# vadimkantorov/convasr

Hardware: AMD Instinct MI355X
Metric: audio-seconds/sec/node (fwd+bwd+CTC) at bs64x15s (higher is better)
Workload: dtype bf16

## Files before the change

### convasr_amd/csrc/conv1x1.hip

```cpp
#include "conv_v2_common.h"

#define C11_THREADS 256
#define C11_BM 128
#define C11_STAGE (2 * C11_BM * ROW_BYTES)

struct C11Args {
	const void* x; const void* w; void* y; const float* bias; double* stats;
	int Cin, Cout, CoutPad;
	int64_t M;
	int accumulate;
};

template <typename I, int NS> __device__ __forceinline__ void conv1x1_tile(const C11Args& p, const int mtile, const int ntile, char* const smem) {
	constexpr int MI = 4, NB = 4;
	const int tid = threadIdx.x, lane = tid & 63;
	const int wave = __builtin_amdgcn_readfirstlane(tid >> 6);
	const int r16 = lane & 15, kb = lane >> 4, wm = wave >> 1, wn = wave & 1;

	const int m0 = mtile * C11_BM, co0 = ntile * BN;
	const int64_t M = p.M;

	const int row_bytes = p.Cin * 2;
	const v4i32 xsrc = make_srd(p.x, (unsigned)(M * row_bytes));
	const v4i32 wsrc = make_srd(p.w, (unsigned)(p.CoutPad * row_bytes));
	const unsigned lds_base = (unsigned)(size_t)(__attribute__((address_space(3))) char*)smem;
	const int n_cib = p.Cin >> 6;

	const int plane = v2s_src_offset(lane, row_bytes);
	auto issue = [&](int cib, int stage) {
		const unsigned dst = lds_base + stage * C11_STAGE;
		const int xbase = m0 * row_bytes + cib * 128, wbase = co0 * row_bytes + cib * 128;
#pragma unroll
		for (int j = 0; j < 4; ++j) {
			const int u = wave + 4 * j;
			dma16(xsrc, __builtin_amdgcn_readfirstlane(dst + u * 1024), xbase + u * 8 * row_bytes + plane);
			dma16(wsrc, __builtin_amdgcn_readfirstlane(dst + C11_BM * ROW_BYTES + u * 1024), wbase + u * 8 * row_bytes + plane);
		}
	};

	f32x4 acc[MI][NB];
#pragma unroll
	for (int i = 0; i < MI; ++i)
#pragma unroll
		for (int j = 0; j < NB; ++j) acc[i][j] = f32x4{0.f, 0.f, 0.f, 0.f};

	typedef unsigned u32x4 __attribute__((ext_vector_type(4)));
	typedef const __attribute__((address_space(3))) u32x4* lds_u4;
	const int kb4 = kb << 4;
	auto lane_off = [&](int row) { return (unsigned)((row << 7) + (kb4 ^ ((row << 4) & 0x60))); };
	const unsigned xa0 = lds_base + lane_off(wm * 64 + r16), wa0 = lds_base + C11_BM * ROW_BYTES + lane_off(wn * 64 + r16);

	if (NS == 2) {
		issue(0, 0);
		asm volatile("s_waitcnt vmcnt(0)" ::: "memory");
	}
	for (int cib = 0; cib < n_cib; ++cib) {
		if (NS == 1) {
			if (cib) __builtin_amdgcn_s_barrier();
			issue(cib, 0);
			asm volatile("s_waitcnt vmcnt(0)" ::: "memory");
		}
		__builtin_amdgcn_s_barrier();
		if (NS == 2 && cib + 1 < n_cib) issue(cib + 1, (cib + 1) & 1);
		const unsigned so = NS == 2 ? (cib & 1) * C11_STAGE : 0u;
#pragma unroll
		for (int ks = 0; ks < 2; ++ks) {
			u32x4 a[MI], b[NB];
			const unsigned xa = (xa0 + so) ^ (ks << 6), wa = (wa0 + so) ^ (ks << 6);
#pragma unroll
			for (int i = 0; i < MI; ++i) { a[i] = *(lds_u4)(size_t)(xa + i * 2048); b[i] = *(lds_u4)(size_t)(wa + i * 2048); }
#pragma unroll
			for (int i = 0; i < MI; ++i)
#pragma unroll
				for (int j = 0; j < NB; ++j) acc[i][j] = Mma16<I>::run(a[i], b[j], acc[i][j]);
		}
		if (NS == 2) asm volatile("s_waitcnt vmcnt(0)" ::: "memory");
	}
	__syncthreads();

	constexpr int OPITCH = BN * 2 + 16;
	char* const otile = smem;
	float* const red = reinterpret_cast<float*>(smem + C11_BM * OPITCH);
	const bool full = m0 + C11_BM <= M;
#pragma unroll
	for (int ni = 0; ni < NB; ++ni) {
		const int col = wn * 64 + ni * 16 + r16, co = co0 + col;
		const float bias = (p.bias && co < p.Cout) ? p.bias[co] : 0.f;
		float s1 = 0.f, s2 = 0.f;
#pragma unroll
		for (int mi = 0; mi < MI; ++mi) {
#pragma unroll
			for (int g = 0; g < 4; ++g) {
				const int row = wm * 64 + mi * 16 + kb * 4 + g;
				const float val = acc[mi][ni][g] + bias;
				if (p.stats && (full || m0 + row < M)) { s1 += val; s2 += val * val; }
				Elem<I>::store(reinterpret_cast<I*>(otile + row * OPITCH) + col, val);
			}
		}
		if (p.stats) {
			s1 += __shfl_xor(s1, 16, 64); s2 += __shfl_xor(s2, 16, 64);
			s1 += __shfl_xor(s1, 32, 64); s2 += __shfl_xor(s2, 32, 64);
			if (kb == 0) { red[(0 * 2 + wm) * BN + col] = s1; red[(1 * 2 + wm) * BN + col] = s2; }
		}
	}
	__syncthreads();
	if (p.stats && tid < BN && co0 + tid < p.Cout) {
		double* const prow = p.stats + (int64_t)mtile * 2 * p.Cout;
		prow[co0 + tid] = (double)red[(0 * 2 + 0) * BN + tid] + (double)red[(0 * 2 + 1) * BN + tid];
		prow[p.Cout + co0 + tid] = (double)red[(1 * 2 + 0) * BN + tid] + (double)red[(1 * 2 + 1) * BN + tid];
	}
	I* const yb = reinterpret_cast<I*>(p.y);
	constexpr int OCH = BN / 8;
#pragma unroll
	for (int it = 0; it < C11_BM * OCH / C11_THREADS; ++it) {
		const int e = tid + it * C11_THREADS, row = e / OCH, ch = e % OCH;
		const int64_t m = (int64_t)m0 + row;
		if (m < M) {
			uint4 val = *reinterpret_cast<const uint4*>(otile + row * OPITCH + ch * 16);
			uint4* const dst = reinterpret_cast<uint4*>(yb + m * p.Cout + co0 + ch * 8);
			if (p.accumulate) {
				float a[8], o[8];
				unpack16<I>(val, a);
				unpack16<I>(*dst, o);
				val = make_uint4(pack16<I>(a[0] + o[0], a[1] + o[1]), pack16<I>(a[2] + o[2], a[3] + o[3]), pack16<I>(a[4] + o[4], a[5] + o[5]), pack16<I>(a[6] + o[6], a[7] + o[7]));
			}
			*dst = val;
		}
	}
}

template <typename I, int NS> __global__ __launch_bounds__(C11_THREADS, NS == 1 ? 4 : 2) void conv1x1_kernel(ConvParams p) {
	extern __shared__ __attribute__((aligned(16))) char smem[];
	const int v = xcd_remap(blockIdx.x, p.total_tiles);
	C11Args a;
	a.x = p.x; a.w = p.w; a.y = p.y; a.bias = p.bias; a.stats = p.stats; a.Cin = p.Cin; a.Cout = p.Cout; a.CoutPad = p.CoutPad; a.M = (int64_t)p.B * p.Tout; a.accumulate = 0;
	conv1x1_tile<I, NS>(a, v / p.n_tiles, v % p.n_tiles, smem);
}

#define C11_MAX_GROUP 12
struct C11Group {
	C11Args prob[C11_MAX_GROUP];
	int first[C11_MAX_GROUP + 1];
	int n_tiles[C11_MAX_GROUP];
	int n;
};

template <typename I, int NS> __global__ __launch_bounds__(C11_THREADS, NS == 1 ? 4 : 2) void conv1x1_grouped_kernel(C11Group g) {
	extern __shared__ __attribute__((aligned(16))) char smem[];
	const int v = xcd_remap(blockIdx.x, g.first[g.n]);
	int q = 0;
#pragma unroll
	for (int i = 1; i < C11_MAX_GROUP; ++i) q += (i < g.n && v >= g.first[i]) ? 1 : 0;
	q = __builtin_amdgcn_readfirstlane(q);
	const int local = v - g.first[q], nt = g.n_tiles[q];
	conv1x1_tile<I, NS>(g.prob[q], local / nt, local % nt, smem);
}

int convasr_conv1x1_try(ConvParams p, int x_dtype, int y_dtype, hipStream_t s, int* rows_out) {
	if (p.K != 1 || p.stride != 1 || p.pad != 0 || p.Tin != p.Tout || (p.Cin & 63) != 0 || (p.Cout & 127) != 0 || p.CoutPad != p.Cout) return 0;
	if (!convasr_is_half(x_dtype) || y_dtype != x_dtype || p.scale || p.act != CONVASR_ACT_NONE || p.xlen || p.bn_y) return 0;
	if (p.debug & 8192) return 0;
	const int64_t M = (int64_t)p.B * p.Tout;
	if (M * p.Cin * 2 >= (1ll << 31) || M * p.Cout * 2 >= (1ll << 31) || (int64_t)p.CoutPad * p.Cin * 2 >= (1ll << 31)) return 0;
	p.n_tiles = p.Cout / BN;
	const int m_tiles = (int)((M + C11_BM - 1) / C11_BM);
	p.total_tiles = m_tiles * p.n_tiles;
	const bool one_stage = (p.Cin < 3 * p.Cout) != ((p.debug & 16384) != 0);
	const size_t epi = (size_t)C11_BM * (BN * 2 + 16) + 4 * BN * sizeof(float);
	const size_t smem = one_stage ? (epi > C11_STAGE ? epi : C11_STAGE) : 2 * (size_t)C11_STAGE;
	const bool f16 = x_dtype == CONVASR_F16;
	const void* kern = one_stage ? (f16 ? (const void*)conv1x1_kernel<f16_t, 1> : (const void*)conv1x1_kernel<bf16_t, 1>) : (f16 ? (const void*)conv1x1_kernel<f16_t, 2> : (const void*)conv1x1_kernel<bf16_t, 2>);
	static unsigned long long set[2][2] = {};
	convasr_allow_160k_lds(kern, set[one_stage][f16]);
	void* args[] = {&p};
	if (hipLaunchKernel(kern, dim3(p.total_tiles), dim3(C11_THREADS), args, smem, s) != hipSuccess) { (void)hipGetLastError(); return 0; }
	if (rows_out) *rows_out = m_tiles;
	return 1;
}

int convasr_conv_debug_bits();
static bool c11_ok(int Cin, int Cout) { return (Cin & 63) == 0 && (Cout & 127) == 0 && Cin > 0 && Cout > 0; }

extern "C" int convasr_conv1x1_grouped(int n, const void* const* x, const void* const* w, void* const* y, const float* const* bias, double* const* stats,
                                       const int* cin, const int* cout, const int* accumulate, int dtype, int B, int T, int* stats_rows, void* stream) {
	CONVASR_CHECK_ARG(n > 0 && n <= C11_MAX_GROUP && x && w && y && cin && cout && B > 0 && T > 0, "conv1x1_grouped: bad arguments (at most %d problems)", C11_MAX_GROUP);
	if (!convasr_is_half(dtype)) return convasr_fail(CONVASR_EUNSUPPORTED, "conv1x1_grouped: dtype %d (16-bit storage only)", dtype);
	const int64_t M = (int64_t)B * T;
	const int m_tiles = (int)((M + C11_BM - 1) / C11_BM);
	for (int i = 0; i < n; ++i) {
		CONVASR_CHECK_ARG(x[i] && w[i] && y[i], "conv1x1_grouped: problem %d has a NULL operand", i);
		if (!c11_ok(cin[i], cout[i]) || M * cin[i] * 2 >= (1ll << 31) || M * cout[i] * 2 >= (1ll << 31) || (int64_t)cout[i] * cin[i] * 2 >= (1ll << 31))
			return convasr_fail(CONVASR_EUNSUPPORTED, "conv1x1_grouped: problem %d (%d -> %d channels, %lld frames) is outside the one-tap kernel's envelope (Cin %% 64, Cout %% 128)", i, cin[i], cout[i], (long long)M);
	}
	const bool f16 = dtype == CONVASR_F16;
	hipStream_t s = (hipStream_t)stream;
	for (int two = 0; two < 2; ++two) {
		C11Group g = {};
		for (int i = 0; i < n; ++i) {
			const bool one_stage = (cin[i] < 3 * cout[i]) != ((convasr_conv_debug_bits() & 16384) != 0);
			if (one_stage == (two != 0)) continue;
			C11Args& a = g.prob[g.n];
			a.x = x[i]; a.w = w[i]; a.y = y[i]; a.bias = bias ? bias[i] : nullptr; a.stats = stats ? stats[i] : nullptr;
			a.Cin = cin[i]; a.Cout = cout[i]; a.CoutPad = cout[i]; a.M = M; a.accumulate = accumulate ? accumulate[i] : 0;
			g.n_tiles[g.n] = cout[i] / BN;
			g.first[g.n + 1] = g.first[g.n] + m_tiles * g.n_tiles[g.n];
			++g.n;
		}
		if (g.n == 0) continue;
		const size_t epi = (size_t)C11_BM * (BN * 2 + 16) + 4 * BN * sizeof(float);
		const size_t smem = two ? 2 * (size_t)C11_STAGE : (epi > C11_STAGE ? epi : C11_STAGE);
		const void* kern = two ? (f16 ? (const void*)conv1x1_grouped_kernel<f16_t, 2> : (const void*)conv1x1_grouped_kernel<bf16_t, 2>) : (f16 ? (const void*)conv1x1_grouped_kernel<f16_t, 1> : (const void*)conv1x1_grouped_kernel<bf16_t, 1>);
		static unsigned long long set[2][2] = {};
		convasr_allow_160k_lds(kern, set[two][f16]);
		void* args[] = {&g};
		if (hipLaunchKernel(kern, dim3(g.first[g.n]), dim3(C11_THREADS), args, smem, s) != hipSuccess) return convasr_fail(CONVASR_ELAUNCH, "conv1x1_grouped: %s", hipGetErrorString(hipGetLastError()));
	}
	if (stats_rows) *stats_rows = m_tiles;
	return 0;
}
```

### convasr_amd/csrc/conv_v2_common.h

```cpp
#pragma once
#include "conv_common.h"

#define V2_BM 256
#define V2_THREADS 512
#define V2_WSLOT (BN * ROW_BYTES)
#define V2S_THREADS (V2_THREADS + 256)

typedef int v4i32 __attribute__((ext_vector_type(4)));

__device__ __forceinline__ v4i32 make_srd(const void* base, unsigned num_bytes) {
	const unsigned long long a = (unsigned long long)base;
	v4i32 d;
	d[0] = __builtin_amdgcn_readfirstlane((int)(unsigned)a);
	d[1] = __builtin_amdgcn_readfirstlane((int)(unsigned)((a >> 32) & 0xffffu));
	d[2] = __builtin_amdgcn_readfirstlane((int)num_bytes);
	d[3] = 0x00020000;
	return d;
}

__device__ __forceinline__ void dma16(const v4i32& srd, unsigned lds_addr, int voff) {
	unsigned keep;
	asm volatile("s_nop 4\n\ts_mov_b32 %0, m0\n\ts_mov_b32 m0, %3\n\ts_nop 0\n\tbuffer_load_dwordx4 %1, %2, 0 offen lds\n\ts_mov_b32 m0, %0"
	             : "=&s"(keep)
	             : "v"(voff), "s"(srd), "s"(lds_addr)
	             : "memory");
}

__device__ __forceinline__ int v2s_swz(int pair) { return (pair & 3) << 1; }
__device__ __forceinline__ int v2s_src_offset(int p, int row_bytes) {
	const int pair = p >> 4, s = p & 15;
	return (2 * pair + (s >> 3)) * row_bytes + (((s & 7) ^ v2s_swz(pair)) << 4);
}
```

### convasr_amd/csrc/conv_v2s.hip

```cpp
#include "conv_v2_common.h"
#include <type_traits>



#ifdef CONVASR_STAMPS
__device__ unsigned long long g_v2s_stamps[256 * 8 * 8];
extern "C" int convasr_debug_read_stamps(unsigned long long* host, int count) {
	return hipMemcpyFromSymbol(host, HIP_SYMBOL(g_v2s_stamps), sizeof(unsigned long long) * count) == hipSuccess ? 0 : -1;
}
#define STAMP(var) { __builtin_amdgcn_sched_barrier(0); asm volatile("s_memtime %0\n\ts_waitcnt lgkmcnt(0)" : "=s"(var) :: "memory"); __builtin_amdgcn_sched_barrier(0); }
#if CONVASR_STAMPS == 1
#define STAMPI(var) STAMP(var)
#else
#define STAMPI(var)
#endif
#else
#define STAMP(var)
#define STAMPI(var)
#endif

template <typename T> struct HalfOnes;
template <> struct HalfOnes<bf16_t> { static constexpr unsigned pair = 0x3F803F80u; };
template <> struct HalfOnes<f16_t> { static constexpr unsigned pair = 0x3C003C00u; };
template <> struct HalfOnes<float> { static constexpr unsigned pair = 0u; };

template <typename I, typename O, int NB, int BNF, int BM_, bool SK = false> __device__ __forceinline__ void v2s_tile(const ConvParams& p, char* smem, const int mtile, const int ntile, const int half, const int bm_full, const int split) {
	constexpr int BN_ = 32 * NB, MI = BM_ / 64, WROWS = 16 * MI;
	constexpr int EPI_OPITCH = BN_ * (int)sizeof(O) + 16, EPI_YOFF = BM_ * EPI_OPITCH + 8 * BN * (int)sizeof(float), EPI_YBYTES = BM_ * BN_ * 2, EPI_LUT = EPI_YOFF + EPI_YBYTES;
	static_assert(BNF != 2 || (EPI_YOFF % 1024 == 0 && EPI_LUT + 4096 <= 160 * 1024), "fused epilogue (form 2): LDS map");
	const int tid = threadIdx.x, lane = tid & 63;
	const int wave = __builtin_amdgcn_readfirstlane(tid >> 6);
	const int r16 = lane & 15, kb = lane >> 4, wm = wave >> 1, wn = wave & 1;

	const int b = mtile / p.m_tiles_per_b, t0 = (mtile % p.m_tiles_per_b) * bm_full;
	const int co0 = ntile * BN + half * BN_;
	const int tin0 = t0 - p.pad;

	const int x_rows = p.x_rows - (bm_full - BM_);
	const int xbytes = x_rows * ROW_BYTES;
	const bool k1 = p.K == 1;
	auto xoff = [&](int c) { return (unsigned)((k1 ? c % 3 : (c & 1)) * xbytes); };
	const unsigned wbase = (k1 ? 3 : 2) * xbytes;
	const int row_bytes = p.Cin * 2;
	const int cib0 = SK ? split * p.cib_per_split : 0;
	const int n_cib = SK ? min(p.cib_per_split, (p.Cin >> 6) - cib0) : (p.Cin >> 6);
	const v4i32 xsrc = make_srd(reinterpret_cast<const char*>(reinterpret_cast<const I*>(p.x) + (int64_t)b * p.Tin * p.Cin) + cib0 * 128, (unsigned)(p.Tin * row_bytes - cib0 * 128));
	const v4i32 wsrc = make_srd(reinterpret_cast<const char*>(p.w) + cib0 * 128, (unsigned)(p.K * p.CoutPad * row_bytes - cib0 * 128));
	const unsigned lds_base = (unsigned)(size_t)(__attribute__((address_space(3))) char*)smem;
	const int x_units = x_rows >> 3;

	const bool loader = wave >= 8;
	const int lw = wave - 8;
	const int xlane = v2s_src_offset(lane, row_bytes);
	auto issue_x = [&](int cib) {
		const unsigned dst = lds_base + xoff(cib);
		const int base = tin0 * row_bytes + cib * 128;
		for (int u = lw; u < x_units; u += 4)
			dma16(xsrc, __builtin_amdgcn_readfirstlane(dst + u * 1024), base + u * 8 * row_bytes + xlane);
	};
	constexpr int PPL = NB;
	int wl[PPL];
#pragma unroll
	for (int j = 0; j < PPL; ++j) wl[j] = v2s_src_offset((lw * PPL + j) * 64 + lane, row_bytes);
	auto issue_w = [&](int q_cib, int q_tap, int slot) {
		const unsigned dst = __builtin_amdgcn_readfirstlane(lds_base + wbase + slot * V2_WSLOT + lw * (1024 * PPL));
		const int base = (q_tap * p.CoutPad + co0) * row_bytes + q_cib * 128;
#pragma unroll
		for (int j = 0; j < PPL; ++j) dma16(wsrc, dst + j * 1024, base + wl[j]);
	};

	f32x4 acc[MI][NB];
#pragma unroll
	for (int i = 0; i < MI; ++i)
#pragma unroll
		for (int j = 0; j < NB; ++j) acc[i][j] = f32x4{0.f, 0.f, 0.f, 0.f};

	typedef unsigned u32x4 __attribute__((ext_vector_type(4)));
	typedef const __attribute__((address_space(3))) u32x4* lds_u4;
	struct Frag { u32x4 a[MI], b[NB]; };
	const int kb4 = kb << 4;
	auto lane_off = [&](int row) { return (unsigned)((row << 7) + (kb4 ^ ((row << 4) & 0x60))); };
	unsigned w0 = lds_base + wbase + lane_off(wn * (16 * NB) + r16);
	asm volatile("" : "+v"(w0));
	auto load_frag = [&](unsigned xs_off, unsigned ws_off, int tap_, int ks, Frag& f) {
		const unsigned xa = (lds_base + xs_off + lane_off(wm * WROWS + r16 + tap_ * p.dil)) ^ (ks << 6);
		const unsigned wa = (w0 + ws_off) ^ (ks << 6);
#ifdef CONVASR_AB_FRAGREADS
		constexpr int RA = (CONVASR_AB_FRAGREADS & 1) ? MI / 2 : MI, RB = (CONVASR_AB_FRAGREADS & 2) ? NB / 2 : NB;
#pragma unroll
		for (int i = 0; i < (MI > NB ? MI : NB); ++i) {
			if (i < RA) f.a[i] = *(lds_u4)(size_t)(xa + i * 2048);
			if (i < RB) f.b[i] = *(lds_u4)(size_t)(wa + i * 2048);
		}
#else
#pragma unroll
		for (int i = 0; i < (MI > NB ? MI : NB); ++i) {
			if (i < MI) f.a[i] = *(lds_u4)(size_t)(xa + i * 2048);
			if (i < NB) f.b[i] = *(lds_u4)(size_t)(wa + i * 2048);
		}
#endif
	};
	auto interleave = [&]() {
#pragma unroll
		for (int i = 0; i < MI + NB; ++i) {
			__builtin_amdgcn_sched_group_barrier(0x100, 1, 0);
			__builtin_amdgcn_sched_group_barrier(0x008, 1, 0);
		}
		if (MI * NB > MI + NB) __builtin_amdgcn_sched_group_barrier(0x008, MI * NB - (MI + NB), 0);
	};
	auto mma_frag = [&](const Frag& f) {
#pragma unroll
		for (int i = 0; i < MI; ++i)
#pragma unroll
			for (int j = 0; j < NB; ++j) acc[i][j] = Mma16<I>::run(f.a[i], f.b[j], acc[i][j]);
	};

// ... 87 lines not shown
#ifdef CONVASR_STAMPS
				acc_issue += tb - ta; acc_work += tc - tb; acc_vm += td - tc; acc_bar += te - td;
#endif
				cib = cib1; pi = pi1;
			}
		};
		if (npb > 1 || k1) main_loop(std::true_type()); else main_loop(std::false_type());
	}

#ifdef CONVASR_STAMPS
	unsigned long long t_epi0 = 0;
	STAMPI(t_epi0)
#endif
	constexpr int OPITCH = EPI_OPITCH;
	char* const otile = smem;
	float* const red = reinterpret_cast<float*>(smem + BM_ * OPITCH);
	const int nvalid = valid_len(p.xlen, b, p.Tout);
	const ActConst ac = act_const(p.act, p.act_lo, p.act_hi), bn_ac = act_const(p.bn_act, p.bn_lo, p.bn_hi);
	constexpr int OEPC_ = 16 / sizeof(O), OCH_ = BN_ / OEPC_, TRIPS = BM_ * OCH_ / V2_THREADS;
	static_assert(BM_ * OCH_ % V2_THREADS == 0, "the store loop covers the tile in whole trips");
	constexpr bool bnf = BNF == 1 && sizeof(O) == 2;
	constexpr bool bnm = BNF == 2 && sizeof(O) == 2;
	typedef typename std::conditional<sizeof(O) == 2, O, I>::type H;
	uint4 ypre[bnf ? TRIPS : 1];
	unsigned gpre[TRIPS];
	if (bnm) {
#pragma unroll
		for (int i = 0; i < TRIPS; ++i) {
			const int e = tid + i * V2_THREADS, row = e / OCH_, t = t0 + row, co = co0 + (e % OCH_) * OEPC_;
			gpre[i] = (t < p.Tout && co < p.Cout) ? p.bn_gate[(((int64_t)b * p.Tout + t) * p.Cout + co) >> 3] : 0u;
		}
		if (tid < 256) {
			unsigned m[4];
#pragma unroll
			for (int i = 0; i < 4; ++i) m[i] = (((tid >> (2 * i)) & 1) ? 0x0000FFFFu : 0u) | (((tid >> (2 * i + 1)) & 1) ? 0xFFFF0000u : 0u);
			*reinterpret_cast<uint4*>(smem + EPI_LUT + tid * 16) = make_uint4(m[0], m[1], m[2], m[3]);
		}
	}
	if (bnf) {
#pragma unroll
		for (int i = 0; i < TRIPS; ++i) {
			const int e = tid + i * V2_THREADS, row = e / OCH_, t = t0 + row, co = co0 + (e % OCH_) * OEPC_;
			ypre[i] = make_uint4(0, 0, 0, 0);
			gpre[i] = 0;
			if (t < p.Tout && co < p.Cout) {
				const int64_t idx = ((int64_t)b * p.Tout + t) * p.Cout + co;
				ypre[i] = *reinterpret_cast<const uint4*>(reinterpret_cast<const H*>(p.bn_y) + idx);
				if (p.bn_gate) gpre[i] = p.bn_gate[idx >> 3];
			}
		}
	}
	auto stage = [&](auto PLAIN_, auto FULL_, auto STATS_, auto LEAKY_) {
		constexpr bool PLAIN = decltype(PLAIN_)::value, FULL = decltype(FULL_)::value, STATS = decltype(STATS_)::value, LEAKY = decltype(LEAKY_)::value;
#pragma unroll
		for (int ni = 0; ni < NB; ++ni) {
			const int col = wn * (16 * NB) + ni * 16 + r16, co = co0 + col;
			const bool cok = co < p.Cout;
			const float bias = (!PLAIN && p.bias && cok) ? p.bias[co] : 0.f;
			const float sc = (!PLAIN && p.scale && cok) ? p.scale[co] : 1.f, sh = (!PLAIN && p.scale && cok) ? p.shift[co] : 0.f;
			float s1 = 0.f, s2 = 0.f;
#pragma unroll
			for (int mi = 0; mi < MI; ++mi) {
#pragma unroll
				for (int g = 0; g < 4; ++g) {
					const int row = wm * WROWS + mi * 16 + kb * 4 + g;
					const int t = t0 + row;
					float val = acc[mi][ni][g];
					if (!PLAIN) val += bias;
					if (STATS && (FULL || t < p.Tout)) { s1 += val; s2 += val * val; }
					if (!PLAIN) {
						val = LEAKY ? apply_act(val * sc + sh, ac) : apply_clamp(val * sc + sh, ac);
						if (t >= nvalid) val = 0.f;
					}
					Elem<O>::store(reinterpret_cast<O*>(otile + row * OPITCH) + col, val);
				}
			}
			if (STATS) {
				s1 += __shfl_xor(s1, 16, 64); s2 += __shfl_xor(s2, 16, 64);
				s1 += __shfl_xor(s1, 32, 64); s2 += __shfl_xor(s2, 32, 64);
				if (kb == 0) { red[(0 * 4 + wm) * BN_ + col] = s1; red[(1 * 4 + wm) * BN_ + col] = s2; }
			}
		}
	};
	{
		typedef std::true_type Y;
		typedef std::false_type N;
		const bool plain = !p.bias && !p.scale && p.act == CONVASR_ACT_NONE && !p.xlen, full = t0 + BM_ <= p.Tout;
		if (!plain) {
			if (ac.leaky) { if (p.stats) stage(N(), N(), Y(), Y()); else stage(N(), N(), N(), Y()); }
			else { if (p.stats) stage(N(), N(), Y(), N()); else stage(N(), N(), N(), N()); }
		}
		else if (p.stats) { if (full) stage(Y(), Y(), Y(), N()); else stage(Y(), N(), Y(), N()); }
		else stage(Y(), Y(), N(), N());
	}
#ifdef CONVASR_STAMPS
	unsigned long long t_e1 = 0, t_e2 = 0, t_e3 = 0;
	STAMPI(t_e1)
#endif
	__syncthreads();
	STAMPI(t_e2)
	if (p.stats && tid < BN_ && co0 + tid < p.Cout) {
		double a = 0, q2 = 0;
#pragma unroll
		for (int m = 0; m < 4; ++m) { a += (double)red[(0 * 4 + m) * BN_ + tid]; q2 += (double)red[(1 * 4 + m) * BN_ + tid]; }
		double* const prow = p.stats + (int64_t)mtile * 2 * p.Cout;
		prow[co0 + tid] = a;
// ... 65 lines not shown
		__syncthreads();
		if (tid < BN_ && co0 + tid < p.Cout) {
			const int chunk = tid >> 3, k = tid & 7;
			double a = 0, q2 = 0;
			for (int j = chunk; j < V2_THREADS; j += OCHUNKS) { a += (double)bnred[j * 17 + k]; q2 += (double)bnred[j * 17 + 8 + k]; }
			double* const prow = p.bn_sums + (int64_t)mtile * 2 * p.Cout;
			prow[co0 + tid] = a;
			prow[p.Cout + co0 + tid] = q2;
		}
	}
	if (bnm) {
		__syncthreads();
		typedef __attribute__((address_space(3))) s16x4* lp;
		typedef unsigned u32x4_ __attribute__((ext_vector_type(4)));
		auto tr8 = [](unsigned addr, unsigned row_stride) {
			const s16x4 lo = __builtin_amdgcn_ds_read_tr16_b64_v4i16((lp)(size_t)addr);
			const s16x4 hi = __builtin_amdgcn_ds_read_tr16_b64_v4i16((lp)(size_t)(addr + 4 * row_stride));
			const uint2 l = __builtin_bit_cast(uint2, lo), h2 = __builtin_bit_cast(uint2, hi);
			u32x4_ r; r[0] = l.x; r[1] = l.y; r[2] = h2.x; r[3] = h2.y;
			return r;
		};
		if (wave < BN_ / 16) {
			const int g4 = lane >> 4, q = (lane >> 2) & 3, pc = lane & 3;
			const unsigned ga = lds_base + (8 * g4 + q) * OPITCH + (16 * wave + 4 * pc) * 2;
			const unsigned ya = lds_base + EPI_YOFF + (8 * g4 + q) * (BN_ * 2) + (16 * wave + 4 * pc) * 2;
			u32x4_ ones; ones[0] = ones[1] = ones[2] = ones[3] = HalfOnes<O>::pair;
			f32x4 a1 = f32x4{0.f, 0.f, 0.f, 0.f}, a2 = f32x4{0.f, 0.f, 0.f, 0.f};
#pragma unroll
			for (int ks = 0; ks < BM_ / 32; ++ks) {
				const u32x4_ gf = tr8(ga + ks * 32 * OPITCH, OPITCH), yf = tr8(ya + ks * 32 * (BN_ * 2), BN_ * 2);
				a1 = Mma16<H>::run(gf, ones, a1);
				a2 = Mma16<H>::run(gf, yf, a2);
			}
			const int c16 = lane & 15, co = co0 + 16 * wave + c16;
			if ((lane >> 4) == (c16 >> 2) && co < p.Cout) {
				const int r = c16 & 3;
				const float s1 = (r == 0 ? a1[0] : r == 1 ? a1[1] : r == 2 ? a1[2] : a1[3]) * gate_scale;
				const float s2 = (r == 0 ? a2[0] : r == 1 ? a2[1] : r == 2 ? a2[2] : a2[3]) * gate_scale;
				double* const prow = p.bn_sums + (int64_t)mtile * 2 * p.Cout;
				prow[co] = (double)s1;
				prow[p.Cout + co] = (double)((s2 - p.bn_mean[co] * s1) * p.bn_invstd[co]);
			}
		}
	}
#ifdef CONVASR_STAMPS
	STAMP(t_end)
	if (blockIdx.x < 256 && lane == 0) {
		unsigned long long* o = g_v2s_stamps + (blockIdx.x * 8 + wave) * 8;
		o[0] = t_loop0 - t_start; o[1] = t_e1 - t_epi0; o[2] = acc_work; o[3] = __builtin_amdgcn_s_memrealtime() - rt_start; o[4] = acc_bar; o[5] = CONVASR_STAMPS == 2 ? rt_start : t_e3 - t_e2; o[6] = t_end - t_e3; o[7] = t_end - t_start;
	}
#endif
}

template <typename I, typename O, int BNF, int BM_, bool SK = false> __global__ __launch_bounds__(V2S_THREADS, 3) void conv1d_igemm_v2s_kernel(ConvParams p) {

	extern __shared__ __attribute__((aligned(16))) char smem[];
	const int bid = blockIdx.x;
	int v, half = 0;
	const bool narrow = bid >= p.full_tiles;
	if (!narrow) v = xcd_remap(bid, p.full_tiles);
	else {
		const int h = xcd_remap(bid - p.full_tiles, 2 * (p.total_tiles - p.full_tiles));
		v = p.full_tiles + (h >> 1);
		half = h & 1;
	}
	int ntile, mtile;
#ifdef CONVASR_AB_BLOCK
	{
		const int sel = (p.debug >> 10) & 7;
		const int MBs[8] = {16, 8, 32, 11, 16, 4, 16, 6}, NTs[8] = {2, 4, 1, 3, 3, 8, 6, 6};
		tile_coords_rt(v, p.B * p.m_tiles_per_b, p.n_tiles, MBs[sel], NTs[sel], mtile, ntile);
	}
#else
	tile_coords(v, p.B * p.m_tiles_per_b, p.n_tiles, mtile, ntile);
#endif
	const bool all_short = p.tail128 == 2;
	const bool tail = all_short || (p.tail128 && (mtile % p.m_tiles_per_b) == p.m_tiles_per_b - 1);
	const int bm_full = all_short ? 128 : BM_;
	const int split = SK ? blockIdx.y : 0;
	if (!tail) {
		if (!narrow) v2s_tile<I, O, 4, BNF, BM_, SK>(p, smem, mtile, ntile, 0, BM_, split);
		else v2s_tile<I, O, 2, BNF, BM_, SK>(p, smem, mtile, ntile, half, BM_, split);
	} else {
		if (!narrow) v2s_tile<I, O, 4, BNF, 128, SK>(p, smem, mtile, ntile, 0, bm_full, split);
		else v2s_tile<I, O, 2, BNF, 128, SK>(p, smem, mtile, ntile, half, bm_full, split);
	}
}

template <typename I, int BM_> static const void* v2s_kernel(int ki) {
	if (ki == 0) return (const void*)conv1d_igemm_v2s_kernel<I, I, 0, BM_>;
	if (ki == 1) return (const void*)conv1d_igemm_v2s_kernel<I, I, 1, BM_>;
	if (ki == 3) return (const void*)conv1d_igemm_v2s_kernel<I, I, 2, BM_>;
	if (ki == 4) return (const void*)conv1d_igemm_v2s_kernel<I, float, 0, BM_, true>;
	return (const void*)conv1d_igemm_v2s_kernel<I, float, 0, BM_>;
}

int convasr_conv1d_v2_try(ConvParams p, int x_dtype, int y_dtype, hipStream_t s, int* m_tiles_out) {
	if (p.stride != 1 || (p.Cin & 63) != 0 || !convasr_is_half(x_dtype) || (y_dtype != x_dtype && y_dtype != CONVASR_F32)) return 0;
	const int n_cu = convasr_cu_count();
#ifdef CONVASR_AB_TILE192
	int bm = (p.debug & 64) ? 192 : V2_BM;
#else
	int bm = V2_BM;
#endif
	bool all_short = false;
	if (bm == V2_BM && !(p.debug & 2048)) {
		const int tiles256 = p.B * ((p.Tout + V2_BM - 1) / V2_BM) * p.n_tiles;
		all_short = (p.debug & 1024) || tiles256 * 4 <= n_cu;
	}
	if (all_short) bm = 128;
	const int xr = (bm - 1) + (p.K - 1) * p.dil + 1;
	p.x_rows = (xr + 15) & ~15;
	const size_t osz = y_dtype == CONVASR_F32 ? 4 : 2;
	size_t smem = 2 * (size_t)p.x_rows * ROW_BYTES + 5 * V2_WSLOT;
	if (p.K == 1) smem = 3 * (size_t)p.x_rows * ROW_BYTES + 3 * V2_WSLOT;
	const bool mfma_sums = p.bn_y && p.bn_gate && !(p.debug & 256);
	const size_t epi = (size_t)bm * (BN * osz + 16) + 8 * BN * sizeof(float) + (p.bn_y ? (mfma_sums ? (size_t)bm * BN * 2 + 4096 : (size_t)V2_THREADS * 17 * sizeof(float)) : 0);
	if (epi > smem) smem = epi;
	if (smem > 160 * 1024) return 0;
	if ((int64_t)p.Tin * p.Cin * 2 >= (1ll << 31) || (int64_t)p.K * p.CoutPad * p.Cin * 2 >= (1ll << 31) || (int64_t)(p.Tout + bm) * p.Cout * 2 >= (1ll << 31)) return 0;
	p.m_tiles_per_b = (p.Tout + bm - 1) / bm;
	p.total_tiles = p.B * p.m_tiles_per_b * p.n_tiles;
	const int tail_rows = p.Tout - (p.m_tiles_per_b - 1) * bm;
	p.tail128 = all_short ? 2 : ((bm == V2_BM && tail_rows <= 128 && !(p.debug & 128)) ? 1 : 0);
	const bool f16 = x_dtype == CONVASR_F16, wide = y_dtype == CONVASR_F32, fused = p.bn_y != nullptr;
	if (fused && wide) return 0;
	if (p.cib_per_split && !wide) return 0;
	const int ki = p.cib_per_split ? 4 : (wide ? 2 : (fused ? (mfma_sums ? 3 : 1) : 0)), bi = bm == 192 ? 1 : 0;
#ifdef CONVASR_AB_TILE192
	const void* kern = f16 ? (bi ? v2s_kernel<f16_t, 192>(ki) : v2s_kernel<f16_t, V2_BM>(ki)) : (bi ? v2s_kernel<bf16_t, 192>(ki) : v2s_kernel<bf16_t, V2_BM>(ki));
#else
	const void* kern = f16 ? v2s_kernel<f16_t, V2_BM>(ki) : v2s_kernel<bf16_t, V2_BM>(ki);
#endif
	static unsigned long long attr_set[2][2][5] = {};
	convasr_allow_160k_lds(kern, attr_set[f16][bi][ki]);
	p.full_tiles = p.total_tiles;
	if (!(p.debug & 32)) {
		const int rest = p.total_tiles % n_cu;
		if (rest > 0 && 2 * rest <= n_cu && ((p.total_tiles - rest) & 7) == 0) p.full_tiles = p.total_tiles - rest;
	}
	const int grid = p.full_tiles + 2 * (p.total_tiles - p.full_tiles);
	const int splits = p.cib_per_split ? ((p.Cin >> 6) + p.cib_per_split - 1) / p.cib_per_split : 1;
	void* args[] = {&p};
	if (hipLaunchKernel(kern, dim3(grid, splits), dim3(V2S_THREADS), args, smem, s) != hipSuccess) { (void)hipGetLastError(); return 0; }
	if (m_tiles_out) *m_tiles_out = p.B * p.m_tiles_per_b;
	return 1;
}
```

Measured before the change: 58530.

## Permute weight rows so each lane stages contiguous output channels in epilogue

Weight rows are loaded into LDS in a permuted order, so each lane's MFMA accumulators hold NB adjacent output channels rather than channels 16 apart. The epilogue can then write 8- or 16-byte packed rows to the staging tile instead of one 2-byte store per element, which cuts LDS store instruction count and bank conflicts. This applies to both the 1x1 and the v2s conv kernels. The old path stays available behind a debug bit, and the v2s fused form 1 is pinned to it. A volatile-barrier square keeps the statistics arithmetic bitwise consistent between paths.

```diff
diff --git a/convasr_amd/csrc/conv1x1.hip b/convasr_amd/csrc/conv1x1.hip
--- a/convasr_amd/csrc/conv1x1.hip
+++ b/convasr_amd/csrc/conv1x1.hip
@@ -1,4 +1,11 @@
 #include "conv_v2_common.h"
+#include <type_traits>
+
+__device__ __forceinline__ float rounded_square(float v) {
+	float q = v * v;
+	asm("" : "+v"(q));
+	return q;
+}
 
 #define C11_THREADS 256
 #define C11_BM 128
@@ -11,7 +18,7 @@
 	int accumulate;
 };
 
-template <typename I, int NS> __device__ __forceinline__ void conv1x1_tile(const C11Args& p, const int mtile, const int ntile, char* const smem) {
+template <typename I, int NS, bool OLDST> __device__ __forceinline__ void conv1x1_tile(const C11Args& p, const int mtile, const int ntile, char* const smem) {
 	constexpr int MI = 4, NB = 4;
 	const int tid = threadIdx.x, lane = tid & 63;
 	const int wave = __builtin_amdgcn_readfirstlane(tid >> 6);
@@ -27,6 +34,7 @@
 	const int n_cib = p.Cin >> 6;
 
 	const int plane = v2s_src_offset(lane, row_bytes);
+	const int wplane = OLDST ? plane : v2s_w_src_offset<4>(lane, row_bytes);
 	auto issue = [&](int cib, int stage) {
 		const unsigned dst = lds_base + stage * C11_STAGE;
 		const int xbase = m0 * row_bytes + cib * 128, wbase = co0 * row_bytes + cib * 128;
@@ -34,7 +42,7 @@
 		for (int j = 0; j < 4; ++j) {
 			const int u = wave + 4 * j;
 			dma16(xsrc, __builtin_amdgcn_readfirstlane(dst + u * 1024), xbase + u * 8 * row_bytes + plane);
-			dma16(wsrc, __builtin_amdgcn_readfirstlane(dst + C11_BM * ROW_BYTES + u * 1024), wbase + u * 8 * row_bytes + plane);
+			dma16(wsrc, __builtin_amdgcn_readfirstlane(dst + C11_BM * ROW_BYTES + u * 1024), wbase + (OLDST ? u * 8 : v2s_w_row<4>(u * 8)) * row_bytes + wplane);
 		}
 	};
 
@@ -82,8 +90,38 @@
 	char* const otile = smem;
 	float* const red = reinterpret_cast<float*>(smem + C11_BM * OPITCH);
 	const bool full = m0 + C11_BM <= M;
-#pragma unroll
-	for (int ni = 0; ni < NB; ++ni) {
+	auto stage = [&](auto STATS_) {
+		constexpr bool STATS = decltype(STATS_)::value;
+		const int col = wn * 64 + NB * r16, co = co0 + col;
+		float bias[NB], s1[NB], s2[NB];
+#pragma unroll
+		for (int j = 0; j < NB; ++j) { bias[j] = (p.bias && co + j < p.Cout) ? p.bias[co + j] : 0.f; s1[j] = s2[j] = 0.f; }
+#pragma unroll
+		for (int mi = 0; mi < MI; ++mi) {
+#pragma unroll
+			for (int g = 0; g < 4; ++g) {
+				const int row = wm * 64 + mi * 16 + kb * 4 + g;
+				float v[NB];
+#pragma unroll
+				for (int j = 0; j < NB; ++j) {
+					v[j] = acc[mi][j][g] + bias[j];
+					if (STATS && (full || m0 + row < M)) { s1[j] += v[j]; s2[j] += rounded_square(v[j]); }
+				}
+				stage_row<I, NB>(otile + row * OPITCH + col * 2, v);
+			}
+		}
+		if (STATS) {
+#pragma unroll
+			for (int j = 0; j < NB; ++j) {
+				s1[j] += __shfl_xor(s1[j], 16, 64); s2[j] += __shfl_xor(s2[j], 16, 64);
+				s1[j] += __shfl_xor(s1[j], 32, 64); s2[j] += __shfl_xor(s2[j], 32, 64);
+				if (kb == 0) { red[(0 * 2 + wm) * BN + col + j] = s1[j]; red[(1 * 2 + wm) * BN + col + j] = s2[j]; }
+			}
+		}
+	};
+	if (!OLDST) { if (p.stats) stage(std::true_type()); else stage(std::false_type()); }
+#pragma unroll
+	for (int ni = 0; OLDST && ni < NB; ++ni) {
 		const int col = wn * 64 + ni * 16 + r16, co = co0 + col;
 		const float bias = (p.bias && co < p.Cout) ? p.bias[co] : 0.f;
 		float s1 = 0.f, s2 = 0.f;
@@ -93,7 +131,7 @@
 			for (int g = 0; g < 4; ++g) {
 				const int row = wm * 64 + mi * 16 + kb * 4 + g;
 				const float val = acc[mi][ni][g] + bias;
-				if (p.stats && (full || m0 + row < M)) { s1 += val; s2 += val * val; }
+				if (p.stats && (full || m0 + row < M)) { s1 += val; s2 += rounded_square(val); }
 				Elem<I>::store(reinterpret_cast<I*>(otile + row * OPITCH) + col, val);
 			}
 		}
@@ -129,12 +167,12 @@
 	}
 }
 
-template <typename I, int NS> __global__ __launch_bounds__(C11_THREADS, NS == 1 ? 4 : 2) void conv1x1_kernel(ConvParams p) {
+template <typename I, int NS, bool OLDST> __global__ __launch_bounds__(C11_THREADS, NS == 1 ? 4 : 2) void conv1x1_kernel(ConvParams p) {
 	extern __shared__ __attribute__((aligned(16))) char smem[];
 	const int v = xcd_remap(blockIdx.x, p.total_tiles);
 	C11Args a;
 	a.x = p.x; a.w = p.w; a.y = p.y; a.bias = p.bias; a.stats = p.stats; a.Cin = p.Cin; a.Cout = p.Cout; a.CoutPad = p.CoutPad; a.M = (int64_t)p.B * p.Tout; a.accumulate = 0;
-	conv1x1_tile<I, NS>(a, v / p.n_tiles, v % p.n_tiles, smem);
+	conv1x1_tile<I, NS, OLDST>(a, v / p.n_tiles, v % p.n_tiles, smem);
 }
 
 #define C11_MAX_GROUP 12
@@ -145,7 +183,7 @@
 	int n;
 };
 
-template <typename I, int NS> __global__ __launch_bounds__(C11_THREADS, NS == 1 ? 4 : 2) void conv1x1_grouped_kernel(C11Group g) {
+template <typename I, int NS, bool OLDST> __global__ __launch_bounds__(C11_THREADS, NS == 1 ? 4 : 2) void conv1x1_grouped_kernel(C11Group g) {
 	extern __shared__ __attribute__((aligned(16))) char smem[];
 	const int v = xcd_remap(blockIdx.x, g.first[g.n]);
 	int q = 0;
@@ -153,8 +191,15 @@
 	for (int i = 1; i < C11_MAX_GROUP; ++i) q += (i < g.n && v >= g.first[i]) ? 1 : 0;
 	q = __builtin_amdgcn_readfirstlane(q);
 	const int local = v - g.first[q], nt = g.n_tiles[q];
-	conv1x1_tile<I, NS>(g.prob[q], local / nt, local % nt, smem);
-}
+	conv1x1_tile<I, NS, OLDST>(g.prob[q], local / nt, local % nt, smem);
+}
+
+template <typename I, bool OLDST> static const void* c11_kernel_st(bool one_stage) { return one_stage ? (const void*)conv1x1_kernel<I, 1, OLDST> : (const void*)conv1x1_kernel<I, 2, OLDST>; }
+static const void* c11_kernel(bool one_stage, bool f16, bool oldst) {
+	if (oldst) return f16 ? c11_kernel_st<f16_t, true>(one_stage) : c11_kernel_st<bf16_t, true>(one_stage);
+	return f16 ? c11_kernel_st<f16_t, false>(one_stage) : c11_kernel_st<bf16_t, false>(one_stage);
+}
+template <typename I, bool OLDST> static const void* c11_grouped_kernel_st(bool two) { return two ? (const void*)conv1x1_grouped_kernel<I, 2, OLDST> : (const void*)conv1x1_grouped_kernel<I, 1, OLDST>; }
 
 int convasr_conv1x1_try(ConvParams p, int x_dtype, int y_dtype, hipStream_t s, int* rows_out) {
 	if (p.K != 1 || p.stride != 1 || p.pad != 0 || p.Tin != p.Tout || (p.Cin & 63) != 0 || (p.Cout & 127) != 0 || p.CoutPad != p.Cout) return 0;
@@ -169,9 +214,10 @@
 	const size_t epi = (size_t)C11_BM * (BN * 2 + 16) + 4 * BN * sizeof(float);
 	const size_t smem = one_stage ? (epi > C11_STAGE ? epi : C11_STAGE) : 2 * (size_t)C11_STAGE;
 	const bool f16 = x_dtype == CONVASR_F16;
-	const void* kern = one_stage ? (f16 ? (const void*)conv1x1_kernel<f16_t, 1> : (const void*)conv1x1_kernel<bf16_t, 1>) : (f16 ? (const void*)conv1x1_kernel<f16_t, 2> : (const void*)conv1x1_kernel<bf16_t, 2>);
-	static unsigned long long set[2][2] = {};
-	convasr_allow_160k_lds(kern, set[one_stage][f16]);
+	const bool oldst = (p.debug & 16) != 0;
+	const void* kern = c11_kernel(one_stage, f16, oldst);
+	static unsigned long long set[2][2][2] = {};
+	convasr_allow_160k_lds(kern, set[one_stage][f16][oldst]);
 	void* args[] = {&p};
 	if (hipLaunchKernel(kern, dim3(p.total_tiles), dim3(C11_THREADS), args, smem, s) != hipSuccess) { (void)hipGetLastError(); return 0; }
 	if (rows_out) *rows_out = m_tiles;
@@ -209,9 +255,10 @@
 		if (g.n == 0) continue;
 		const size_t epi = (size_t)C11_BM * (BN * 2 + 16) + 4 * BN * sizeof(float);
 		const size_t smem = two ? 2 * (size_t)C11_STAGE : (epi > C11_STAGE ? epi : C11_STAGE);
-		const void* kern = two ? (f16 ? (const void*)conv1x1_grouped_kernel<f16_t, 2> : (const void*)conv1x1_grouped_kernel<bf16_t, 2>) : (f16 ? (const void*)conv1x1_grouped_kernel<f16_t, 1> : (const void*)conv1x1_grouped_kernel<bf16_t, 1>);
-		static unsigned long long set[2][2] = {};
-		convasr_allow_160k_lds(kern, set[two][f16]);
+		const bool oldst = (convasr_conv_debug_bits() & 16) != 0;
+		const void* kern = oldst ? (f16 ? c11_grouped_kernel_st<f16_t, true>(two) : c11_grouped_kernel_st<bf16_t, true>(two)) : (f16 ? c11_grouped_kernel_st<f16_t, false>(two) : c11_grouped_kernel_st<bf16_t, false>(two));
+		static unsigned long long set[2][2][2] = {};
+		convasr_allow_160k_lds(kern, set[two][f16][oldst]);
 		void* args[] = {&g};
 		if (hipLaunchKernel(kern, dim3(g.first[g.n]), dim3(C11_THREADS), args, smem, s) != hipSuccess) return convasr_fail(CONVASR_ELAUNCH, "conv1x1_grouped: %s", hipGetErrorString(hipGetLastError()));
 	}
diff --git a/convasr_amd/csrc/conv_v2_common.h b/convasr_amd/csrc/conv_v2_common.h
--- a/convasr_amd/csrc/conv_v2_common.h
+++ b/convasr_amd/csrc/conv_v2_common.h
@@ -31,3 +31,15 @@
 	const int pair = p >> 4, s = p & 15;
 	return (2 * pair + (s >> 3)) * row_bytes + (((s & 7) ^ v2s_swz(pair)) << 4);
 }
+template <int NB> __device__ __forceinline__ int v2s_w_row(int R) { return (R / (16 * NB)) * (16 * NB) + NB * (R & 15) + ((R >> 4) % NB); }
+template <int NB> __device__ __forceinline__ int v2s_w_src_offset(int p, int row_bytes) {
+	const int pair = p >> 4, s = p & 15;
+	return v2s_w_row<NB>(2 * pair + (s >> 3)) * row_bytes + (((s & 7) ^ v2s_swz(pair)) << 4);
+}
+template <typename O, int N> __device__ __forceinline__ void stage_row(char* dst, const float (&v)[N]) {
+	static_assert(N == 2 || N == 4, "stage_row: two or four channels");
+	if constexpr (sizeof(O) == 2 && N == 4) *reinterpret_cast<uint2*>(dst) = make_uint2(pack16<O>(v[0], v[1]), pack16<O>(v[2], v[3]));
+	else if constexpr (sizeof(O) == 2) *reinterpret_cast<unsigned*>(dst) = pack16<O>(v[0], v[1]);
+	else if constexpr (N == 4) *reinterpret_cast<float4*>(dst) = make_float4(v[0], v[1], v[2], v[3]);
+	else *reinterpret_cast<float2*>(dst) = make_float2(v[0], v[1]);
+}
diff --git a/convasr_amd/csrc/conv_v2s.hip b/convasr_amd/csrc/conv_v2s.hip
--- a/convasr_amd/csrc/conv_v2s.hip
+++ b/convasr_amd/csrc/conv_v2s.hip
@@ -24,7 +24,7 @@
 template <> struct HalfOnes<f16_t> { static constexpr unsigned pair = 0x3C003C00u; };
 template <> struct HalfOnes<float> { static constexpr unsigned pair = 0u; };
 
-template <typename I, typename O, int NB, int BNF, int BM_, bool SK = false> __device__ __forceinline__ void v2s_tile(const ConvParams& p, char* smem, const int mtile, const int ntile, const int half, const int bm_full, const int split) {
+template <typename I, typename O, int NB, int BNF, int BM_, bool SK = false, bool OLDST = false> __device__ __forceinline__ void v2s_tile(const ConvParams& p, char* smem, const int mtile, const int ntile, const int half, const int bm_full, const int split) {
 	constexpr int BN_ = 32 * NB, MI = BM_ / 64, WROWS = 16 * MI;
 	constexpr int EPI_OPITCH = BN_ * (int)sizeof(O) + 16, EPI_YOFF = BM_ * EPI_OPITCH + 8 * BN * (int)sizeof(float), EPI_YBYTES = BM_ * BN_ * 2, EPI_LUT = EPI_YOFF + EPI_YBYTES;
 	static_assert(BNF != 2 || (EPI_YOFF % 1024 == 0 && EPI_LUT + 4096 <= 160 * 1024), "fused epilogue (form 2): LDS map");
@@ -61,7 +61,7 @@
 	constexpr int PPL = NB;
 	int wl[PPL];
 #pragma unroll
-	for (int j = 0; j < PPL; ++j) wl[j] = v2s_src_offset((lw * PPL + j) * 64 + lane, row_bytes);
+	for (int j = 0; j < PPL; ++j) wl[j] = OLDST ? v2s_src_offset((lw * PPL + j) * 64 + lane, row_bytes) : v2s_w_src_offset<NB>((lw * PPL + j) * 64 + lane, row_bytes);
 	auto issue_w = [&](int q_cib, int q_tap, int slot) {
 		const unsigned dst = __builtin_amdgcn_readfirstlane(lds_base + wbase + slot * V2_WSLOT + lw * (1024 * PPL));
 		const int base = (q_tap * p.CoutPad + co0) * row_bytes + q_cib * 128;
@@ -255,6 +255,48 @@
 	}
 	auto stage = [&](auto PLAIN_, auto FULL_, auto STATS_, auto LEAKY_) {
 		constexpr bool PLAIN = decltype(PLAIN_)::value, FULL = decltype(FULL_)::value, STATS = decltype(STATS_)::value, LEAKY = decltype(LEAKY_)::value;
+		if (!OLDST) {
+			const int col = wn * (16 * NB) + NB * r16, co = co0 + col;
+			float bias[NB], sc[NB], sh[NB], s1[NB], s2[NB];
+#pragma unroll
+			for (int j = 0; j < NB; ++j) {
+				const bool cok = co + j < p.Cout;
+				bias[j] = (!PLAIN && p.bias && cok) ? p.bias[co + j] : 0.f;
+				sc[j] = (!PLAIN && p.scale && cok) ? p.scale[co + j] : 1.f;
+				sh[j] = (!PLAIN && p.scale && cok) ? p.shift[co + j] : 0.f;
+				s1[j] = s2[j] = 0.f;
+			}
+#pragma unroll
+			for (int mi = 0; mi < MI; ++mi) {
+#pragma unroll
+				for (int g = 0; g < 4; ++g) {
+					const int row = wm * WROWS + mi * 16 + kb * 4 + g;
+					const int t = t0 + row;
+					float v[NB];
+#pragma unroll
+					for (int j = 0; j < NB; ++j) {
+						float val = acc[mi][j][g];
+						if (!PLAIN) val += bias[j];
+						if (STATS && (FULL || t < p.Tout)) { s1[j] += val; s2[j] += val * val; }
+						if (!PLAIN) {
+							val = LEAKY ? apply_act(val * sc[j] + sh[j], ac) : apply_clamp(val * sc[j] + sh[j], ac);
+							if (t >= nvalid) val = 0.f;
+						}
+						v[j] = val;
+					}
+					stage_row<O, NB>(otile + row * OPITCH + col * (int)sizeof(O), v);
+				}
+			}
+			if (STATS) {
+#pragma unroll
+				for (int j = 0; j < NB; ++j) {
+					s1[j] += __shfl_xor(s1[j], 16, 64); s2[j] += __shfl_xor(s2[j], 16, 64);
+					s1[j] += __shfl_xor(s1[j], 32, 64); s2[j] += __shfl_xor(s2[j], 32, 64);
+					if (kb == 0) { red[(0 * 4 + wm) * BN_ + col + j] = s1[j]; red[(1 * 4 + wm) * BN_ + col + j] = s2[j]; }
+				}
+			}
+			return;
+		}
 #pragma unroll
 		for (int ni = 0; ni < NB; ++ni) {
 			const int col = wn * (16 * NB) + ni * 16 + r16, co = co0 + col;
@@ -426,7 +468,7 @@
 #endif
 }
 
-template <typename I, typename O, int BNF, int BM_, bool SK = false> __global__ __launch_bounds__(V2S_THREADS, 3) void conv1d_igemm_v2s_kernel(ConvParams p) {
+template <typename I, typename O, int BNF, int BM_, bool SK = false, bool OLDST = false> __global__ __launch_bounds__(V2S_THREADS, 3) void conv1d_igemm_v2s_kernel(ConvParams p) {
 
 	extern __shared__ __attribute__((aligned(16))) char smem[];
 	const int bid = blockIdx.x;
@@ -453,21 +495,22 @@
 	const int bm_full = all_short ? 128 : BM_;
 	const int split = SK ? blockIdx.y : 0;
 	if (!tail) {
-		if (!narrow) v2s_tile<I, O, 4, BNF, BM_, SK>(p, smem, mtile, ntile, 0, BM_, split);
-		else v2s_tile<I, O, 2, BNF, BM_, SK>(p, smem, mtile, ntile, half, BM_, split);
+		if (!narrow) v2s_tile<I, O, 4, BNF, BM_, SK, OLDST>(p, smem, mtile, ntile, 0, BM_, split);
+		else v2s_tile<I, O, 2, BNF, BM_, SK, OLDST>(p, smem, mtile, ntile, half, BM_, split);
 	} else {
-		if (!narrow) v2s_tile<I, O, 4, BNF, 128, SK>(p, smem, mtile, ntile, 0, bm_full, split);
-		else v2s_tile<I, O, 2, BNF, 128, SK>(p, smem, mtile, ntile, half, bm_full, split);
+		if (!narrow) v2s_tile<I, O, 4, BNF, 128, SK, OLDST>(p, smem, mtile, ntile, 0, bm_full, split);
+		else v2s_tile<I, O, 2, BNF, 128, SK, OLDST>(p, smem, mtile, ntile, half, bm_full, split);
 	}
 }
 
-template <typename I, int BM_> static const void* v2s_kernel(int ki) {
-	if (ki == 0) return (const void*)conv1d_igemm_v2s_kernel<I, I, 0, BM_>;
-	if (ki == 1) return (const void*)conv1d_igemm_v2s_kernel<I, I, 1, BM_>;
-	if (ki == 3) return (const void*)conv1d_igemm_v2s_kernel<I, I, 2, BM_>;
-	if (ki == 4) return (const void*)conv1d_igemm_v2s_kernel<I, float, 0, BM_, true>;
-	return (const void*)conv1d_igemm_v2s_kernel<I, float, 0, BM_>;
+template <typename I, int BM_, bool OLDST> static const void* v2s_kernel_st(int ki) {
+	if (ki == 0) return (const void*)conv1d_igemm_v2s_kernel<I, I, 0, BM_, false, OLDST>;
+	if (ki == 1) return (const void*)conv1d_igemm_v2s_kernel<I, I, 1, BM_, false, true>;
+	if (ki == 3) return (const void*)conv1d_igemm_v2s_kernel<I, I, 2, BM_, false, OLDST>;
+	if (ki == 4) return (const void*)conv1d_igemm_v2s_kernel<I, float, 0, BM_, true, OLDST>;
+	return (const void*)conv1d_igemm_v2s_kernel<I, float, 0, BM_, false, OLDST>;
 }
+template <typename I, int BM_> static const void* v2s_kernel(int ki, bool oldst) { return oldst ? v2s_kernel_st<I, BM_, true>(ki) : v2s_kernel_st<I, BM_, false>(ki); }
 
 int convasr_conv1d_v2_try(ConvParams p, int x_dtype, int y_dtype, hipStream_t s, int* m_tiles_out) {
 	if (p.stride != 1 || (p.Cin & 63) != 0 || !convasr_is_half(x_dtype) || (y_dtype != x_dtype && y_dtype != CONVASR_F32)) return 0;
@@ -500,14 +543,15 @@
 	const bool f16 = x_dtype == CONVASR_F16, wide = y_dtype == CONVASR_F32, fused = p.bn_y != nullptr;
 	if (fused && wide) return 0;
 	if (p.cib_per_split && !wide) return 0;
+	const bool oldst = (p.debug & 16) != 0;
 	const int ki = p.cib_per_split ? 4 : (wide ? 2 : (fused ? (mfma_sums ? 3 : 1) : 0)), bi = bm == 192 ? 1 : 0;
 #ifdef CONVASR_AB_TILE192
-	const void* kern = f16 ? (bi ? v2s_kernel<f16_t, 192>(ki) : v2s_kernel<f16_t, V2_BM>(ki)) : (bi ? v2s_kernel<bf16_t, 192>(ki) : v2s_kernel<bf16_t, V2_BM>(ki));
+	const void* kern = f16 ? (bi ? v2s_kernel<f16_t, 192>(ki, oldst) : v2s_kernel<f16_t, V2_BM>(ki, oldst)) : (bi ? v2s_kernel<bf16_t, 192>(ki, oldst) : v2s_kernel<bf16_t, V2_BM>(ki, oldst));
 #else
-	const void* kern = f16 ? v2s_kernel<f16_t, V2_BM>(ki) : v2s_kernel<bf16_t, V2_BM>(ki);
-#endif
-	static unsigned long long attr_set[2][2][5] = {};
-	convasr_allow_160k_lds(kern, attr_set[f16][bi][ki]);
+	const void* kern = f16 ? v2s_kernel<f16_t, V2_BM>(ki, oldst) : v2s_kernel<bf16_t, V2_BM>(ki, oldst);
+#endif
+	static unsigned long long attr_set[2][2][5][2] = {};
+	convasr_allow_160k_lds(kern, attr_set[f16][bi][ki][oldst]);
 	p.full_tiles = p.total_tiles;
 	if (!(p.debug & 32)) {
 		const int rest = p.total_tiles % n_cu;
diff --git a/scratch/staging_banks.py b/scratch/staging_banks.py
--- /dev/null
+++ b/scratch/staging_banks.py
@@ -0,0 +1,37 @@
+
+
+def w_row(R, nb):
+	return (R // (16 * nb)) * (16 * nb) + nb * (R % 16) + (R // 16) % nb
+
+
+def worst(pitch, esize, nb, bm):
+	mi_n, wrows = bm // 64, bm // 4
+	nbytes = nb * esize
+	group = {4: 32, 8: 16, 16: 8}[nbytes]
+	w = 0
+	for wm in range(4):
+		for wn in range(2):
+			for mi in range(mi_n):
+				for g in range(4):
+					for g0 in range(0, 64, group):
+						banks = {}
+						for lane in range(g0, g0 + group):
+							r16, kb = lane & 15, lane >> 4
+							a = (wm * wrows + mi * 16 + kb * 4 + g) * pitch + (wn * 16 * nb + nb * r16) * esize
+							assert a % nbytes == 0
+							for d in range(nbytes // 4):
+								banks.setdefault((a // 4 + d) % 32, set()).add(a // 4 + d)
+						w = max(w, max(len(v) for v in banks.values()))
+	return w
+
+
+if __name__ == '__main__':
+	for nb in (4, 2):
+		assert sorted(w_row(R, nb) for R in range(32 * nb)) == list(range(32 * nb))
+		assert all(w_row(R, nb) // (16 * nb) == R // (16 * nb) for R in range(32 * nb))
+		assert all(w_row(wn * 16 * nb + 16 * j + r, nb) == wn * 16 * nb + nb * r + j for wn in range(2) for j in range(nb) for r in range(16))
+	for esize, name in ((2, '16-bit tile'), (4, 'fp32 tile')):
+		for nb, bm in ((4, 256), (4, 128), (2, 256), (2, 128)):
+			row = 32 * nb * esize
+			res = {pad: worst(row + pad, esize, nb, bm) for pad in range(0, 80, 16)}
+			print(f'{name}, {bm} x {32 * nb} tile, {nb * esize}-byte writes: worst multiplicity by pad ' + ', '.join(f'+{pad}: {v}' for pad, v in res.items()) + f' | shipped +16: {res[16]}')
diff --git a/scratch/stamps_staging.py b/scratch/stamps_staging.py
--- /dev/null
+++ b/scratch/stamps_staging.py
@@ -0,0 +1,55 @@
+import os, sys, ctypes, json
+sys.path.insert(0, os.path.dirname(os.path.dirname(os.path.abspath(__file__))))
+import numpy as np, torch
+from convasr_amd import ops, _lib
+d = torch.device('cuda:0'); dt = torch.bfloat16
+lib = _lib.load()
+B, T = 64, 751
+
+
+def forward(cin, cout, k):
+	x = ops.as_cl(torch.randn(B, cin, T, device = d).clamp_(0, 20), dt)
+	wp = ops.pack_weight(torch.randn(cout, cin, k, device = d) / (cin * k) ** 0.5, dt, _lib.PACK_FWD)
+	st = ops.ConvStats(cout, B, T, d)
+	return lambda: ops.conv1d(x, wp, cout, k, 1, 1, k // 2, stats = st)
+
+
+def dgrad_plain(cin, cout, k):
+	dy = ops.as_cl(torch.randn(B, cout, T, device = d), dt)
+	_, wd = ops.pack_weight(torch.randn(cout, cin, k, device = d) / (cin * k) ** 0.5, dt, None)
+	return lambda: ops.conv1d(dy, wd, cin, k, 1, 1, k - 1 - k // 2)
+
+
+def dgrad_fused(cin, cout, k):
+	dy = ops.as_cl(torch.randn(B, cout, T, device = d), dt)
+	_, wd = ops.pack_weight(torch.randn(cout, cin, k, device = d) / (cin * k) ** 0.5, dt, None)
+	yb = ops.as_cl(torch.randn(B, cin, T, device = d) * 3 + 1, dt)
+	sc, sh, mean, istd = (torch.rand(cin, device = d) + 0.5 for _ in range(4))
+	xl = torch.ones(B, device = d)
+	act = (_lib.ACT_HARDTANH, 0.0, 20.0)
+	gate = torch.zeros(B * T * cin // 8, dtype = torch.uint8, device = d)
+	ops.bn_act(yb, sc, sh, act, xlen = xl, dropout_p = 0.2, seed = 1, offset = 0, gate = gate)
+	sums = ops.ConvStats(cin, B, T, d)
+	return lambda: ops.conv1d_dgrad_bn_reduce(dy, wd, cin, k, 1, k - 1 - k // 2, yb, sc, sh, mean, istd, act, 0.2, 1, 0, xl, sums, gate = gate)
+
+
+LAUNCHES = [('768->768 k11 forward + statistics', forward(768, 768, 11), 0), ('256->256 k11 forward + statistics', forward(256, 256, 11), 0),
+            ('768->768 k11 dgrad + fused BN-backward sums (form 2)', dgrad_fused(768, 768, 11), 0), ('one-tap dgrad 1024 -> 896 (conv_v2s.hip, bit 8192)', dgrad_plain(896, 1024, 1), 8192)]
+names = ['prologue', 'staging', 'lds+mfma', 'realtime_100MHz', 'barrier_wait', 'stats', 'store_loop', 'tile']
+out = {}
+for label, run, bits in LAUNCHES:
+	for arm, arm_bits in (('old', 16), ('new', 0), ('old', 16), ('new', 0)):
+		prev = lib.convasr_debug_set_conv_v2(1 | ((bits | arm_bits) << 8))
+		try:
+			for _ in range(10): run()
+			torch.cuda.synchronize()
+		finally:
+			lib.convasr_debug_set_conv_v2(prev)
+		buf = np.zeros(256 * 8 * 8, dtype = np.uint64)
+		assert lib.convasr_debug_read_stamps(buf.ctypes.data_as(ctypes.c_void_p), buf.size) == 0
+		m = buf.reshape(256, 8, 8).astype(np.float64).mean(axis = (0, 1))
+		rec = {n: float(v) for n, v in zip(names, m)}
+		out.setdefault(label, {}).setdefault(arm, []).append(rec)
+		print(f'{label} | {arm}: prologue {m[0]:.0f} staging {m[1]:.0f} stats+barrier {m[5]:.0f} store loop (+ fused sums) {m[6]:.0f} | tile {m[7]:.0f} cycles, {m[7] / max(m[3], 1) * 0.1:.3f} GHz in-kernel', flush = True)
+if len(sys.argv) > 1:
+	json.dump(out, open(sys.argv[1], 'w'), indent = 1)
```

Result: no change. 58690 (median of 3 runs) (+0.3%).
